# ReaganCardoza/Physics-Based-Ray-Tracing

Hardware: AMD Instinct MI355X
Metric: Msamples/s on cbox.xml 512x512 x 256 spp (radiance, path max_depth 6) (higher is better)
Workload: dtype f32

## Files before the change

### physics-based-ray-tracing_amd/csrc/device_scene.h

```cpp
#pragma once
#include "../../include/pbrt_hip.h"
#include "device_math.h"

struct DevNode4 {
    float org[3];
    uint32_t exps;
    uint32_t child[4];
    uint32_t qlo[3];
    uint32_t qhi[3];
    uint32_t pad[2];
};
struct DevLeafPrim {
    float g[9];
    uint32_t meta;
};
#define LDS_AS __attribute__((address_space(3)))
#define PRIV_AS __attribute__((address_space(5)))
typedef uint32_t __attribute__((ext_vector_type(4))) u32x4;
typedef uint32_t __attribute__((ext_vector_type(2))) u32x2;
struct NodeQ {
    u32x4 w0, w1, w2;
    u32x2 w3;
};
struct LeafQ {
    u32x2 a, b, c, d, e;
};
struct TreeGlobal {
    const DevNode4 *nodes;
    const DevLeafPrim *lprims;
    DEV NodeQ node(uint32_t n) const {
        const DevNode4 *np = nodes + n;
        NodeQ q;
        q.w0 = *reinterpret_cast<const u32x4 *>(&np->org[0]);
        q.w1 = *reinterpret_cast<const u32x4 *>(&np->child[0]);
        q.w2 = *reinterpret_cast<const u32x4 *>(&np->qlo[0]);
        q.w3 = *reinterpret_cast<const u32x2 *>(&np->qhi[1]);
        return q;
    }
    DEV NodeQ node_boxes(uint32_t n) const {
        const DevNode4 *np = nodes + n;
        NodeQ q;
        q.w0 = *reinterpret_cast<const u32x4 *>(&np->org[0]);
        q.w1 = q.w0;
        q.w2 = *reinterpret_cast<const u32x4 *>(&np->qlo[0]);
        q.w3 = *reinterpret_cast<const u32x2 *>(&np->qhi[1]);
        return q;
    }
    DEV uint32_t child(uint32_t n, uint32_t slot) const { return nodes[n].child[slot]; }
    DEV LeafQ leaf(uint32_t s) const {
        const u32x2 *q = reinterpret_cast<const u32x2 *>(&lprims[s]);
        return {q[0], q[1], q[2], q[3], q[4]};
    }
};
struct TreeLds {
    const LDS_AS uint32_t *img;
    uint32_t plane;
    uint32_t leaf_off;
    DEV NodeQ node(uint32_t n) const {
        const LDS_AS char *b = reinterpret_cast<const LDS_AS char *>(img);
        const uint32_t a = n * 16u;
        NodeQ q;
        q.w0 = *reinterpret_cast<const LDS_AS u32x4 *>(b + a);
        q.w1 = *reinterpret_cast<const LDS_AS u32x4 *>(b + plane + a);
        q.w2 = *reinterpret_cast<const LDS_AS u32x4 *>(b + 2u * plane + a);
        q.w3 = *reinterpret_cast<const LDS_AS u32x2 *>(b + 3u * plane + n * 8u);
        return q;
    }
    DEV NodeQ node_boxes(uint32_t n) const {
        const LDS_AS char *b = reinterpret_cast<const LDS_AS char *>(img);
        const uint32_t a = n * 16u;
        NodeQ q;
        q.w0 = *reinterpret_cast<const LDS_AS u32x4 *>(b + a);
        q.w1 = q.w0;
        q.w2 = *reinterpret_cast<const LDS_AS u32x4 *>(b + 2u * plane + a);
        q.w3 = *reinterpret_cast<const LDS_AS u32x2 *>(b + 3u * plane + n * 8u);
        return q;
    }
    DEV uint32_t child(uint32_t n, uint32_t slot) const {
        const LDS_AS char *b = reinterpret_cast<const LDS_AS char *>(img);
        return *reinterpret_cast<const LDS_AS uint32_t *>(b + plane + n * 16u + slot * 4u);
    }
    DEV LeafQ leaf(uint32_t s) const {
        const LDS_AS u32x2 *q = reinterpret_cast<const LDS_AS u32x2 *>(reinterpret_cast<const LDS_AS char *>(img) + leaf_off + s * 40u);
        return {q[0], q[1], q[2], q[3], q[4]};
    }
};
#define LDS_IMAGE_NODE_BYTES 56u
#define BVH_LEAF 0x80000000u
#define BVH_SENT 0xffffffffu

struct DevScene {
    const pbrt_prim *prims;
    const DevLeafPrim *lprims;
    const DevNode4 *nodes;
    const pbrt_material *mats;
    const pbrt_emitter *emitters;
    const uint32_t *light_prims;
    const float *light_cdf;
    const pbrt_prim *prims_by_id;
    const pbrt_prim *occ_prims;
    uint32_t n_occ;
    const float *vnormals;
    uint32_t n_prims, n_nodes, n_emitters, n_mats, n_light_prims;
};

struct Hit {
    float t, u, v;
    uint32_t prim;
    uint32_t slot;
};

DEV V3 g3(const pbrt_prim &P, int i) { return {P.g[i], P.g[i + 1], P.g[i + 2]}; }

DEV bool cone_hit(const pbrt_prim &P, V3 o, V3 d, float tmax, float *t, float *flag) {
    const V3 r0 = g3(P, 0), r1 = g3(P, 4), r2 = g3(P, 8);
    const V3 oo = {dot(r0, o) + P.g[3], dot(r1, o) + P.g[7], dot(r2, o) + P.g[11]};
    const V3 dd = {dot(r0, d), dot(r1, d), dot(r2, d)};
    const float ow = 1.0f - oo.z;
    const float A = fma_(dd.x, dd.x, fma_(dd.y, dd.y, -(dd.z * dd.z)));
    const float b = fma_(oo.x, dd.x, fma_(oo.y, dd.y, ow * dd.z));
    const float C = fma_(oo.x, oo.x, fma_(oo.y, oo.y, -(ow * ow)));
    const float disc = fma_(b, b, -(A * C));
    float best = tmax;
    float fl = 0.0f;
    bool found = false;
    if (disc >= 0.0f) {
        const float q = -(b + copysignf(sqrtf(disc), b));
        const float ta = q / A, tb = C / q;
        const float za = fma_(ta, dd.z, oo.z), zb = fma_(tb, dd.z, oo.z);
        if (ta >= 0.0f && ta <= best && za >= 0.0f && za <= 1.0f) {
            best = ta;
            found = true;
        }
        if (tb >= 0.0f && tb <= best && zb >= 0.0f && zb <= 1.0f && (!found || tb < best)) {
            best = tb;
            found = true;
        }
    }
    const float tc = -oo.z / dd.z;
    const float x = fma_(tc, dd.x, oo.x), y = fma_(tc, dd.y, oo.y);
    if (tc >= 0.0f && tc <= best && fma_(x, x, y * y) <= 1.0f && (!found || tc < best)) {
        best = tc;
        fl = 1.0f;
        found = true;
    }
    *t = best;
    *flag = fl;
    return found;
}

DEV bool cylinder_hit(const pbrt_prim &P, V3 o, V3 d, float tmax, float *t) {
    const V3 r0 = g3(P, 0), r1 = g3(P, 4), r2 = g3(P, 8);
    const V3 oo = {dot(r0, o) + P.g[3], dot(r1, o) + P.g[7], dot(r2, o) + P.g[11]};
    const V3 dd = {dot(r0, d), dot(r1, d), dot(r2, d)};
    const float A = fma_(dd.x, dd.x, dd.y * dd.y);
    const float b = fma_(oo.x, dd.x, oo.y * dd.y);
    const float C = fma_(oo.x, oo.x, fma_(oo.y, oo.y, -1.0f));
    const float disc = fma_(b, b, -(A * C));
    if (!(disc >= 0.0f)) return false;
    const float q = -(b + copysignf(sqrtf(disc), b));
    const float ta = q / A, tb = C / q;
    const float za = fma_(ta, dd.z, oo.z), zb = fma_(tb, dd.z, oo.z);
    float best = tmax;
    bool found = false;
    if (ta >= 0.0f && ta <= best && za >= 0.0f && za <= 1.0f) {
        best = ta;
        found = true;
    }
    if (tb >= 0.0f && tb <= best && zb >= 0.0f && zb <= 1.0f && (!found || tb < best)) {
        best = tb;
        found = true;
    }
    *t = best;
    return found;
}

DEV bool sphere_hit(V3 c, float r, V3 o, V3 d, float tmax, float *t) {
    V3 f = o - c;
    float bp = -dot(f, d);
    V3 perp = madd(d, bp, f);
    float disc = fma_(r, r, -dot(perp, perp));
    if (!(disc >= 0.0f)) return false;
    float sq = sqrtf(disc);
    float q = bp + copysignf(sq, bp);
    float cc = fma_(-r, r, dot(f, f));
    float t0 = cc / q, t1 = q;
    float tn = fminf(t0, t1), tf = fmaxf(t0, t1);
    if (!(tn <= tmax && tf >= 0.0f)) return false;
    if (tn < 0.0f && tf > tmax) return false;
    *t = tn < 0.0f ? tf : tn;
    return true;
}
DEV bool planar_hit(bool triangle, V3 v0, V3 e1, V3 e2, V3 o, V3 d, float tmax, float *t, float *u, float *v) {
    V3 pvec = cross(d, e2);
    float det = dot(e1, pvec);
    V3 tvec = o - v0;
    V3 qvec = cross(tvec, e1);
    float us = dot(tvec, pvec), vs = dot(d, qvec), ts = dot(e2, qvec);
    const uint32_t sgn = __float_as_uint(det) & 0x80000000u;
    det = __uint_as_float(__float_as_uint(det) ^ sgn);
    us = __uint_as_float(__float_as_uint(us) ^ sgn);
    vs = __uint_as_float(__float_as_uint(vs) ^ sgn);
    ts = __uint_as_float(__float_as_uint(ts) ^ sgn);
    const float lim = triangle ? us + vs : fmaxf(us, vs);
    const bool ok = (det > 0.0f) & (us >= 0.0f) & (vs >= 0.0f) & (ts >= 0.0f) & (lim <= det);
    if (!ok) return false;
    float inv = 1.0f / det;
    float tt = ts * inv;
    if (!(tt <= tmax)) return false;
    *t = tt;
    *u = us * inv;
    *v = vs * inv;
    return true;
}
template <bool CYL = true>
DEV bool prim_hit(const pbrt_prim &P, V3 o, V3 d, float tmax, float *t, float *u, float *v) {
    const uint32_t type = P.type;
    if (type == PBRT_PRIM_SPHERE) {
        *u = 0.0f;
        *v = 0.0f;
        return sphere_hit(g3(P, 0), P.g[3], o, d, tmax, t);
    }
    if (type == PBRT_PRIM_TRIANGLE || type == PBRT_PRIM_PARALLELOGRAM)
        return planar_hit(type == PBRT_PRIM_TRIANGLE, g3(P, 0), g3(P, 3), g3(P, 6), o, d, tmax, t, u, v);
    if (type == PBRT_PRIM_CONE) {
        *v = 0.0f;
        return cone_hit(P, o, d, tmax, t, u);
    }
    if (CYL && type == PBRT_PRIM_CYLINDER) {
        *u = 0.0f;
        *v = 0.0f;
        return cylinder_hit(P, o, d, tmax, t);
    }
    return false;
}

DEV pbrt_prim load_prim_uniform(const pbrt_prim *p) {
    typedef uint32_t __attribute__((ext_vector_type(4))) u32x4;
    typedef const u32x4 __attribute__((address_space(4))) *cptr;
    struct Raw {
        u32x4 q[4];
    };
    static_assert(sizeof(Raw) == sizeof(pbrt_prim), "pbrt_prim is 16 dwords");
    cptr q = (cptr)(uintptr_t)p;
    Raw r = {{q[0], q[1], q[2], q[3]}};
    return __builtin_bit_cast(pbrt_prim, r);
}

template <bool ANY, bool SEGMENT = false, bool CONES = true>
DEV bool brute_intersect(const DevScene &sc, V3 o, V3 d, float tmax, Hit *h) {
    bool found = false;
    float bn = 0.0f, bd = 1.0f, bu = 0.0f, bv = 0.0f;
    uint32_t bp = 0xffffffffu;
    const pbrt_prim *list = (ANY && SEGMENT) ? sc.occ_prims : sc.prims;
    const uint32_t n_list = (uint32_t)__builtin_amdgcn_readfirstlane((int)((ANY && SEGMENT) ? sc.n_occ : sc.n_prims));
    if (n_list == 0) return false;
    pbrt_prim nxt = load_prim_uniform(list);
    for (uint32_t i = 0; i < n_list; ++i) {
        const pbrt_prim P = nxt;
        nxt = load_prim_uniform(list + min(i + 1, n_list - 1));
        const uint32_t type = P.type;
        bool ok;
        float num, den, us, vs;
        if (type == PBRT_PRIM_SPHERE || (CONES && (type == PBRT_PRIM_CONE || type == PBRT_PRIM_CYLINDER))) {
            float t, u, v;
            ok = prim_hit(P, o, d, tmax, &t, &u, &v);
            num = t;
            den = 1.0f;
            us = u;
            vs = 0.0f;
        } else {
            V3 v0 = g3(P, 0), e1 = g3(P, 3), e2 = g3(P, 6);
            V3 pvec = cross(d, e2);
            float det = dot(e1, pvec);
            V3 tvec = o - v0;
            V3 qvec = cross(tvec, e1);
            us = dot(tvec, pvec);
            vs = dot(d, qvec);
            float ts = dot(e2, qvec);
            const bool neg = det < 0.0f;
            det = neg ? -det : det;
            us = neg ? -us : us;
            vs = neg ? -vs : vs;
            ts = neg ? -ts : ts;
            ok = (det > 0.0f) & (fminf(fminf(us, vs), ts) >= 0.0f) & (ts <= tmax * det);
            if (type == PBRT_PRIM_TRIANGLE)
                ok = ok & (us + vs <= det);
            else
                ok = ok & (fmaxf(us, vs) <= det);
            num = ts;
            den = det;
        }
        if (ANY) {
            found = found | ok;
            if (__builtin_amdgcn_ballot_w64(!found) == 0) break;
        } else {
            const bool better = ok & (!found | (num * bd < bn * den));
            bn = better ? num : bn;
            bd = better ? den : bd;
            bu = better ? us : bu;
            bv = better ? vs : bv;
            bp = better ? i : bp;
            found = found | better;
        }
    }
    if (!ANY && found) {
        float inv = 1.0f / bd;
        h->t = bn * inv;
        h->u = bu * inv;
        h->v = bv * inv;
        h->prim = bp;
        h->slot = bp;
    }
    return found;
}

struct BoxRay {
    V3 o, inv;
};
DEV BoxRay make_box_ray(V3 o, V3 d) {
    const float tiny = 1e-18f;
    const V3 ds = {fabsf(d.x) < tiny ? copysignf(tiny, d.x) : d.x, fabsf(d.y) < tiny ? copysignf(tiny, d.y) : d.y,
                   fabsf(d.z) < tiny ? copysignf(tiny, d.z) : d.z};
    return {o, {__builtin_amdgcn_rcpf(ds.x), __builtin_amdgcn_rcpf(ds.y), __builtin_amdgcn_rcpf(ds.z)}};
}

#define BVH_STK_OVF 30
#define BVH_STK_MAX (BVH_STK_OVF + 2)
struct BvhStack {
    LDS_AS uint32_t *col;
    uint32_t shift;
    uint32_t n_rows;
};
struct BvhCursor {
    uint32_t cur, tos, sp;
};
struct BvhOvf {
    uint32_t m[BVH_STK_OVF];
    DEV PRIV_AS uint32_t *at(uint32_t i) { return (PRIV_AS uint32_t *)(&m[0]) + min(i, (uint32_t)BVH_STK_OVF - 1u); }
};
DEV void bvh_push(const BvhStack &st, BvhCursor &c, BvhOvf &ovf, bool on, uint32_t entry) {
    if (on) {
        if (c.sp < st.n_rows)
            st.col[c.sp << st.shift] = c.tos;
        else
            *ovf.at(c.sp - st.n_rows) = c.tos;
        c.sp += 1u;
        c.tos = entry;
    }
}
template <typename Tree>
DEV uint32_t bvh_pop(const Tree &tr, const BvhStack &st, BvhCursor &c, BvhOvf &ovf) {
    const uint32_t e = c.tos;
    if (e == BVH_SENT) return BVH_SENT;
    const uint32_t ref = tr.child(e >> 8, e & 3u);
    const uint32_t n = (e >> 6) & 3u;
    if (n > 1u) {
        c.tos = (e & 0xffffff00u) | ((n - 1u) << 6) | ((e & 0x3fu) >> 2);
    } else {
        const uint32_t sp1 = c.sp - 1u;
        if (sp1 < st.n_rows)
            c.tos = st.col[sp1 << st.shift];
        else
            c.tos = *ovf.at(sp1 - st.n_rows);
        c.sp = sp1;
    }
    return ref;
}

template <bool MISS_SLOT = false>
DEV void bvh_child_keys(const NodeQ &q, const BoxRay &r, float best, uint32_t key[4]) {
    const uint32_t exps = q.w0.w;
    const float Ax = __uint_as_float((exps & 0xffu) << 23) * r.inv.x, Ay = __uint_as_float(((exps >> 8) & 0xffu) << 23) * r.inv.y,
                Az = __uint_as_float(((exps >> 16) & 0xffu) << 23) * r.inv.z;
    const float Bx = (__uint_as_float(q.w0.x) - r.o.x) * r.inv.x, By = (__uint_as_float(q.w0.y) - r.o.y) * r.inv.y,
                Bz = (__uint_as_float(q.w0.z) - r.o.z) * r.inv.z;
    const bool nx = r.inv.x < 0.0f, ny = r.inv.y < 0.0f, nz = r.inv.z < 0.0f;
    const uint32_t qnx = nx ? q.w2.w : q.w2.x, qfx = nx ? q.w2.x : q.w2.w;
    const uint32_t qny = ny ? q.w3.x : q.w2.y, qfy = ny ? q.w2.y : q.w3.x;
    const uint32_t qnz = nz ? q.w3.y : q.w2.z, qfz = nz ? q.w2.z : q.w3.y;
#pragma unroll
    for (int k = 0; k < 4; ++k) {
        const float tnx = fma_((float)((qnx >> (8 * k)) & 0xffu), Ax, Bx), tfx = fma_((float)((qfx >> (8 * k)) & 0xffu), Ax, Bx);
        const float tny = fma_((float)((qny >> (8 * k)) & 0xffu), Ay, By), tfy = fma_((float)((qfy >> (8 * k)) & 0xffu), Ay, By);
        const float tnz = fma_((float)((qnz >> (8 * k)) & 0xffu), Az, Bz), tfz = fma_((float)((qfz >> (8 * k)) & 0xffu), Az, Bz);
        const float tn = fmaxf(fmaxf(tnx, tny), fmaxf(tnz, 0.0f));
        const float tf = fminf(fminf(tfx, tfy), fminf(tfz, best));
        key[k] = (tn <= tf) ? ((__float_as_uint(tn) & ~3u) | (uint32_t)k) : (MISS_SLOT ? (0xfffffffcu | (uint32_t)k) : 0xffffffffu);
    }
}

DEV void bvh_cex(uint32_t &ka, uint32_t &kb) {
    const uint32_t lo = min(ka, kb), hi = max(ka, kb);
    ka = lo;
    kb = hi;
// ... 556 lines not shown
```

### physics-based-ray-tracing_amd/csrc/pbrt_api.hip

```cpp
#include <hip/hip_runtime.h>

#include <cmath>
#include <cstdarg>
#include <cstdio>
#include <cstring>
#include <map>
#include <numeric>
#include <string>
#include <vector>

#include "bvh_build.h"
#include "kernels_us.h"
#include "kernels_wavefront.h"
#include "kernels_us_wavefront.h"
#include "kernels_beamform.h"
#include "workspace.h"

static std::string g_ctxless_error;

struct HipAlloc {
    static const int out_of_memory = hipErrorOutOfMemory;
    static int alloc(void **p, size_t bytes) {
        const hipError_t e = hipMalloc(p, bytes);
        if (e != hipSuccess) (void)hipGetLastError();
        return e;
    }
    static void free(void *p) { (void)hipFree(p); }
    static const char *error_string(int e) { return hipGetErrorString((hipError_t)e); }
};

#define PIN_GUARD_OFFSET ((2 + MAX_DEPTH_STATS) * REDUCE_SLICES * 8)
#define PIN_BYTES (PIN_GUARD_OFFSET + 4096)

struct pbrt_ctx {
    int device = 0;
    int n_cu = 256;
    hipStream_t stream = nullptr;
    hipStream_t st_trace = nullptr, st_shade = nullptr;
    uint32_t split_s = 0;
    std::vector<hipEvent_t> sync_ev;
    std::string err;
    pbrt_stats stats{};
    Workspace<HipAlloc> work;
    uint64_t call_seq = 0;
    std::vector<hipEvent_t> ev_pool;
    struct PendingAcq {
        bool active = false, streams = false, tab0 = false;
        bool scaled = true;
        bool timed = true;
        size_t n_ev = 0;
        uint32_t passes = 0, launches = 0;
        uint64_t samples = 0, nchan = 0;
    } pend;
    void *pinned = nullptr;
    unsigned long long *pin_stats() { return (unsigned long long *)pinned; }
    uint32_t *pin_guard() { return (uint32_t *)((char *)pinned + PIN_GUARD_OFFSET); }
    uint64_t us_rows_gen = 0;
    size_t us_rows_bytes = 0;
    std::vector<float> us_tab_host;
    uint64_t us_tab_gen = 0;
    bool profiling = false;
    hipEvent_t img_ev[8] = {nullptr, nullptr, nullptr, nullptr, nullptr, nullptr, nullptr, nullptr};
    uint32_t img_mask = 0;
    uint64_t img_das_bytes = 0;
    size_t env_lds_attr = 0;
    uint32_t env_taps_n = 0;
    uint64_t env_taps_gen = 0;
    uint64_t wf_guard_gen = 0;
    bool img_event(int i) { return img_ev[i] || hipEventCreate(&img_ev[i]) == hipSuccess; }
    hipEvent_t ev0 = nullptr, ev1 = nullptr;
    uint32_t lds_limit = 0;
    bool recording = false, rec_failed = false;
    std::string rec_msg;

    int fail(int code, const char *fmt, ...) {
        char buf[1024];
        va_list ap;
        va_start(ap, fmt);
        vsnprintf(buf, sizeof buf, fmt, ap);
        va_end(ap);
        err = buf;
        if (recording && !rec_failed) {
            rec_failed = true;
            rec_msg = buf;
        }
        return code;
    }
    int refuse(const char *what) {
        err = std::string("a recording is open on this context (pbrt_ctx_record_begin): ") + what;
        return PBRT_E_INVALID;
    }
    void *buf(const char *name, size_t bytes) {
        void *p = work.get(name, bytes, call_seq, recording);
        if (!p) fail(PBRT_E_NOMEM, "%s", work.error.c_str());
// ... 294 lines not shown
    NEED(c, d->n_prims > 0 && d->prims && d->n_materials > 0 && d->materials);
    NEED(c, d->n_emitters == 0 || d->emitters);
    NEED(c, d->n_light_prims == 0 || (d->light_prims && d->light_cdf));
    for (uint32_t i = 0; i < d->n_prims; ++i) {
        const pbrt_prim &p = d->prims[i];
        if (p.type > PBRT_PRIM_CYLINDER) return c->fail(PBRT_E_UNSUPPORTED, "primitive %u: type %u is not supported", i, p.type);
        if (p.type == PBRT_PRIM_CONE) {
            double cc[3], ca[3], cb[3], cx[3];
            if (!cone_world_frame(p, cc, ca, cb, cx))
                return c->fail(PBRT_E_INVALID, "primitive %u: cone needs an invertible, finite world -> object matrix", i);
        }
        if (p.type == PBRT_PRIM_CYLINDER) {
            double c0[3], c1[3], ca[3], cb[3];
            if (!cylinder_world_frame(p, c0, c1, ca, cb))
                return c->fail(PBRT_E_INVALID, "primitive %u: cylinder needs an invertible, finite world -> object matrix", i);
        }
        if (p.material >= d->n_materials) return c->fail(PBRT_E_INVALID, "primitive %u: material out of range", i);
        if (p.emitter >= 0 && (uint32_t)p.emitter >= d->n_emitters)
            return c->fail(PBRT_E_INVALID, "primitive %u: emitter out of range", i);
    }
    for (uint32_t i = 0; i < d->n_materials; ++i)
        if (int rc = check_material(c, d->materials[i], i)) return rc;
    for (uint32_t i = 0; i < d->n_emitters; ++i) {
        const pbrt_emitter &e = d->emitters[i];
        if (e.type == PBRT_EMIT_AREA) {
            if (e.count == 0 || e.first + e.count > d->n_light_prims)
                return c->fail(PBRT_E_INVALID, "emitter %u: light primitive range out of bounds", i);
            for (uint32_t k = 0; k < e.count; ++k) {
                uint32_t pi = d->light_prims[e.first + k];
                if (pi >= d->n_prims || d->prims[pi].type == PBRT_PRIM_SPHERE || d->prims[pi].type == PBRT_PRIM_CONE ||
                    d->prims[pi].type == PBRT_PRIM_CYLINDER)
                    return c->fail(PBRT_E_UNSUPPORTED, "emitter %u: area lights need triangle/parallelogram primitives", i);
            }
        } else if (e.type != PBRT_EMIT_POINT) {
            return c->fail(PBRT_E_INVALID, "emitter %u: unknown type", i);
        }
    }
    if (d->vertex_normals)
        for (size_t i = 0; i < (size_t)d->n_prims * 9; ++i)
            if (!std::isfinite(d->vertex_normals[i])) return c->fail(PBRT_E_INVALID, "vertex_normals: entry %zu is not finite", i);
    HIPCHK(c, hipSetDevice(c->device));
    pbrt_scene *s = new pbrt_scene();
    s->ctx = c;
    int rc;
    const pbrt_prim *d_prims_by_id = nullptr;
#define UP(call)               \
    if ((rc = (call)) != 0) {  \
        pbrt_scene_destroy(s); \
        return rc;             \
    }
    UP(upload(s, d->prims, d->n_prims, &d_prims_by_id));
    s->ds.prims_by_id = d_prims_by_id;
    s->ds.n_prims = d->n_prims;
    const pbrt_material *dm = nullptr;
    UP(upload(s, d->materials, d->n_materials, &dm));
    s->ds.mats = dm;
    s->d_mats = const_cast<pbrt_material *>(dm);
    s->n_mats = s->ds.n_mats = d->n_materials;
    for (uint32_t i = 0; i < d->n_materials; ++i) s->mat_types.push_back(d->materials[i].type);
    UP(upload(s, d->emitters, d->n_emitters, &s->ds.emitters));
    s->ds.n_emitters = d->n_emitters;
    UP(upload(s, d->light_prims, d->n_light_prims, &s->ds.light_prims));
    UP(upload(s, d->light_cdf, d->n_light_prims, &s->ds.light_cdf));
    s->ds.n_light_prims = d->n_light_prims;
    NEED(c, d->accel <= PBRT_ACCEL_BVH_GLOBAL);
    const bool want_bvh = d->accel == PBRT_ACCEL_BVH || d->accel == PBRT_ACCEL_BVH_GLOBAL ||
                          (d->accel == PBRT_ACCEL_AUTO && d->n_prims > 32);
    if (!want_bvh) {
        s->ds.prims = d_prims_by_id;
        s->ds.lprims = nullptr;
        s->ds.nodes = nullptr;
        s->ds.n_nodes = 0;
        bool small = d->n_prims <= TAB_MAX && d->n_materials <= TAB_MAX && d->n_emitters <= TAB_MAX;
        for (uint32_t i = 0; i < d->n_prims; ++i)
            if (d->prims[i].type == PBRT_PRIM_CONE || d->prims[i].type == PBRT_PRIM_CYLINDER)
                small = false;
        if (d->vertex_normals) small = false;
        if (d->vertex_normals) UP(upload(s, d->vertex_normals, (size_t)d->n_prims * 9, &s->ds.vnormals));
        s->small_tables = small;
        s->accel_kernel = small ? ACCEL_K_BRUTE : ACCEL_K_BRUTE_BIG;
        std::vector<pbrt_prim> occ = find_occluders(d);
        UP(upload(s, occ.data(), occ.size(), &s->ds.occ_prims));
        s->ds.n_occ = (uint32_t)occ.size();
    } else {
        HostBvh bvh;
        const bool sure_global = !c->lds_limit || (size_t)d->n_prims * sizeof(DevLeafPrim) > c->lds_limit || d->accel == PBRT_ACCEL_BVH_GLOBAL;
        build_bvh(d->prims, d->n_prims, &bvh, sure_global ? BVH_CTRAV_GLOBAL : BVH_CTRAV);
        HostBvh4 b4;
        to_bvh4(bvh, &b4);
        if (b4.depth > BVH_STK_MAX || b4.nodes.size() >= (1u << 24) - 1u || d->n_prims >= (1u << 27)) {
            pbrt_scene_destroy(s);
            return c->fail(PBRT_E_UNSUPPORTED, "BVH depth %u / %zu nodes exceed the traversal state", b4.depth, b4.nodes.size());
        }
        std::vector<HostLeafPrim> lp;
        make_leaf_prims(d->prims, bvh.order, &lp);
        static_assert(sizeof(HostLeafPrim) == sizeof(DevLeafPrim) && sizeof(DevLeafPrim) == 40, "leaf record layout");
        static_assert(sizeof(HostNode4) == sizeof(DevNode4) && sizeof(DevNode4) == 64, "node layout");
        s->ds.prims = d_prims_by_id;
        const DevLeafPrim *dl = nullptr;
        UP(upload(s, reinterpret_cast<const DevLeafPrim *>(lp.data()), lp.size(), &dl));
        s->ds.lprims = dl;
        if (d->vertex_normals) UP(upload(s, d->vertex_normals, (size_t)d->n_prims * 9, &s->ds.vnormals));
        const DevNode4 *dn = nullptr;
        UP(upload(s, reinterpret_cast<const DevNode4 *>(b4.nodes.data()), b4.nodes.size(), &dn));
        s->ds.nodes = dn;
        s->ds.n_nodes = (uint32_t)b4.nodes.size();
        s->bvh_depth = b4.depth;
        s->curved = false;
        for (uint32_t i = 0; i < d->n_prims; ++i) {
            if (d->prims[i].type != PBRT_PRIM_TRIANGLE && d->prims[i].type != PBRT_PRIM_PARALLELOGRAM) s->curved = true;
            if (d->prims[i].type == PBRT_PRIM_CYLINDER) s->cylinders = true;
        }
        const size_t lds = b4.nodes.size() * LDS_IMAGE_NODE_BYTES + (size_t)d->n_prims * sizeof(DevLeafPrim);
        if (c->lds_limit && lds + BVH_STK_DW(SEG_BVH) * 4 + 1024 <= c->lds_limit && d->accel != PBRT_ACCEL_BVH_GLOBAL) {
            s->accel_kernel = ACCEL_K_BVH_LDS;
            s->lds_bytes = (uint32_t)((lds + 15) & ~size_t(15));
        } else {
            s->accel_kernel = ACCEL_K_BVH_GLOBAL;
        }
    }
#undef UP
    scene_set_glossy(s);
    *out = s;
    return PBRT_OK;
}

int pbrt_scene_update_material(pbrt_scene *s, uint32_t index, const pbrt_material *m) {
    if (!s) return PBRT_E_INVALID;
    pbrt_ctx *c = s->ctx;
    NEED(c, m && index < s->n_mats);
    NOT_RECORDING(c);
    if (int rc = check_material(c, *m, index)) return rc;
    HIPCHK(c, hipSetDevice(c->device));
    HIPCHK(c, hipMemcpyAsync(s->d_mats + index, m, sizeof *m, hipMemcpyHostToDevice, c->stream));
    s->mat_types[index] = m->type;
    scene_set_glossy(s);
    return PBRT_OK;
}

int pbrt_scene_destroy(pbrt_scene *s) {
    if (!s) return PBRT_OK;
    NOT_RECORDING(s->ctx);
    (void)hipSetDevice(s->ctx->device);
    (void)ctx_settle(s->ctx);
    (void)hipStreamSynchronize(s->ctx->stream);
    s->ctx->work.invalidate_recordings();
    for (void *p : s->allocs) (void)hipFree(p);
    delete s;
    return PBRT_OK;
}

}

struct Switches {
    bool wf_packet = true;
    uint32_t wf_split_s = 0, wf_split_parts = 1;
    bool us_generic_kernel = false, us_emit_fused = true, env_general = false;
    int us_emit_permute = 1;
#ifdef PBRT_DIAG
    uint32_t pair_merge = 0;
    bool us_fused_bvh = false;
#endif
};
static Switches read_switches() {
    static const Switches once = [] {
        Switches w;
// ... 581 lines not shown
    const uint32_t W = cam->film_w, H = cam->film_h;
    NEED(c, W > 0 && H > 0 && f->crop_w > 0 && f->crop_h > 0);
    NEED(c, (uint64_t)f->crop_x + f->crop_w <= W && (uint64_t)f->crop_y + f->crop_h <= H);
    NEED(c, f->spp > 0 && f->max_depth > 0 && f->filter <= PBRT_FILTER_GAUSSIAN);
    NEED(c, (uint64_t)W * H <= 0xffffffffull);
    HIPCHK(c, hipSetDevice(c->device));
    const bool brute = s->accel_kernel == ACCEL_K_BRUTE || s->accel_kernel == ACCEL_K_BRUTE_BIG;
    const bool wavefront = !brute && !(f->flags & PBRT_FILM_NO_HIT_POOL);
    const Switches sw = read_switches();
#ifndef PBRT_DIAG
    if ((f->flags & (PBRT_FILM_REGEN | PBRT_FILM_WALK_SET)) || (!brute && (f->flags & PBRT_FILM_NO_HIT_POOL)))
        return c->fail(PBRT_E_UNSUPPORTED, "PBRT_FILM_REGEN / PBRT_FILM_WALK_FROM / PBRT_FILM_NO_HIT_POOL select diagnostic launch "
                                           "structures: build libpbrt_hip_diag.so (make -C csrc diag)");
#endif
    int rc = set_lds_attr(s);
    if (rc) return rc;
    const uint32_t R = f->filter == PBRT_FILTER_BOX ? 0 : (f->filter == PBRT_FILTER_TENT ? 1 : 2);
    const uint32_t rx0 = f->crop_x > R ? f->crop_x - R : 0, ry0 = f->crop_y > R ? f->crop_y - R : 0;
    const uint32_t rx1 = std::min(f->crop_x + f->crop_w + R, W), ry1 = std::min(f->crop_y + f->crop_h + R, H);
    const uint32_t rw = rx1 - rx0, rh = ry1 - ry0;
    const uint64_t npix_r = (uint64_t)rw * rh;
    const uint64_t film_px = (uint64_t)f->crop_w * f->crop_h;
    const uint64_t pass_paths = f->pass_paths ? f->pass_paths
                                              : default_pass_paths(c, wavefront, brute ? (64u << 20) : (16u << 20), 16 + 2 * N_STATE * 4);
    static_assert(WF_REGION == REGION_SEGS_BVH * SEG_BVH, "both BVH launch structures cut a pass into the same regions");
    const uint32_t REGION = rad_region_segs(s->accel_kernel) * seg_threads(s->accel_kernel);
    WfBufs wfb{};
    float *Lhome = nullptr;
    auto alloc_pass = [&](uint32_t cap, uint32_t nseg) -> int {
        NEED(c, wavefront || (uint64_t)cap * N_STATE * 4 < 0xffffffffull);
        if (wavefront) NEED(c, cap < WF_DEAD);
        Lhome = (float *)c->buf("Lhome", (size_t)cap * 16);
        return Lhome && (!wavefront || wf_alloc(c, cap, nseg, &wfb)) ? PBRT_OK : PBRT_E_NOMEM;
    };
    PassShape ps;
    if ((rc = size_pass(c, pass_paths, f->pass_paths != 0, f->spp, npix_r, REGION, true, alloc_pass, &ps)) != 0) return rc;
    const uint32_t s_pass = ps.per_pass, cap = ps.cap, nseg = ps.nseg;
    WfPlan wfp;
    if (wavefront) {
        wfp = wf_plan(s, sw);
        if ((rc = wf_set_attr(s, wfp)) != 0) return rc;
    }
    float *stA = wavefront ? (float *)wfb.stA : nullptr;
    float *stB = wavefront ? (float *)wfb.stB : nullptr;
    const bool repack = !brute && !wavefront && rad_wave_private(s->accel_kernel) && !(f->flags & PBRT_FILM_NO_REPACK);
    float *stC = repack ? (float *)c->buf("stateC", (size_t)cap * N_STATE * 4) : nullptr;
    const uint32_t n_own = nseg * rad_owners_per_region(s->accel_kernel);
    uint32_t *segA = (uint32_t *)c->buf("segA", (size_t)n_own * 4);
    uint32_t *segB = (uint32_t *)c->buf("segB", (size_t)n_own * 4);
    uint32_t *segC = repack ? (uint32_t *)c->buf("segC", (size_t)n_own * 4) : nullptr;
    uint32_t *offs = repack ? (uint32_t *)c->buf("seg_offs", (size_t)n_own * 4) : nullptr;
    uint32_t *quota = repack ? (uint32_t *)c->buf("seg_quota", 64) : nullptr;
    float *acc = (float *)c->buf("film_acc", film_px * 16);
    unsigned long long *dstats = (unsigned long long *)c->buf("stats", (2 + 2 * MAX_DEPTH_STATS) * 8);
    const uint32_t n_rows = nseg * (wavefront ? WF_SHADE_THREADS / 64u : rad_rows_per_region(s->accel_kernel));
    const uint32_t stat_rows = 2 + (uint32_t)std::min<uint64_t>(f->max_depth, MAX_DEPTH_STATS);
    const size_t segstats_bytes = (size_t)stat_rows * n_rows * 8;
    unsigned long long *segstats = (unsigned long long *)c->buf("segstats", (size_t)(2 + 2 * MAX_DEPTH_STATS) * n_rows * 8);
    if (!segstats) return PBRT_E_NOMEM;
    if (!Lhome || !segA || !segB || !acc || !dstats) return PBRT_E_NOMEM;
    const uint32_t hit_rows = wavefront ? stat_rows - 2 : 0;
    if (repack && (!stC || !segC || !offs || !quota)) return PBRT_E_NOMEM;
    hipStream_t st = c->stream;
    HIPCHK(c, hipMemsetAsync(acc, 0, film_px * 16, st));
    HIPCHK(c, hipMemsetAsync(dstats, 0, (2 + 2 * MAX_DEPTH_STATS) * 8, st));
    HIPCHK(c, hipMemsetAsync(segstats, 0, segstats_bytes, st));
    if (hit_rows) HIPCHK(c, hipMemsetAsync(segstats + (size_t)HIT_ROW0 * n_rows, 0, (size_t)hit_rows * n_rows * 8, st));
    HIPCHK(c, hipEventRecord(c->ev0, st));
    PassTimer timer{c};
    uint32_t passes = 0, launches = 0;
    const bool plan_was_learnt = brute && s->plan_hint_valid;
    uint32_t plan = !brute ? 0u
                    : (f->flags & PBRT_FILM_FUSE_PLAN_SET) ? ((f->flags >> 8) & 0xffu)
                    : (s->plan_hint_valid ? s->plan_hint : PBRT_DEFAULT_FUSE_PLAN);
    constexpr uint32_t PROBE_SPP = 2;
    const bool probe = brute && !s->plan_hint_valid && f->spp >= 8 * PROBE_SPP && s_pass >= PROBE_SPP &&
                       !(f->flags & (PBRT_FILM_FUSE_PLAN_SET | PBRT_FILM_WALK_SET | PBRT_FILM_REGEN));
    const uint32_t walk_from = (f->flags & PBRT_FILM_WALK_SET) ? ((f->flags >> 17) & 0xffu) : PBRT_DEFAULT_WALK_FROM;
    RadArgs base{};
    base.sc = s->ds;
    if ((f->flags & PBRT_FILM_NO_OCCLUDER_PRUNING) && base.sc.occ_prims) {
        base.sc.occ_prims = base.sc.prims;
        base.sc.n_occ = base.sc.n_prims;
    }
    base.cam = *cam;
    base.Lhome = Lhome;
    base.stats = segstats;
    base.stat_stride = n_rows;
    base.cap = cap;
    base.state_cap = cap;
    base.max_depth = f->max_depth;
    base.rr_depth = f->rr_depth;
    base.seed = f->seed;
    base.key_mode = 0;
    base.rx0 = rx0;
    base.ry0 = ry0;
    base.rw = rw;
    base.npix_r = (uint32_t)npix_r;
    base.tile_rows = rh & ~7u;
    base.div_npix = make_fastdiv(base.npix_r);
    base.div_rw = make_fastdiv(rw);
    const std::initializer_list<uint32_t> probes = {0u, 1u, rw - 1, rw, rw + 1, base.npix_r - 1, base.npix_r, base.npix_r + 1, cap - 1, cap, 0xffffffffu};
    NEED(c, fastdiv_exact(base.div_npix, base.npix_r, probes) && fastdiv_exact(base.div_rw, rw, probes));
    base.film_w = W;
    base.film_h = H;
    base.lds_bytes = s->lds_bytes;
    FilmArgs fa{};
    fa.Lhome = Lhome;
    fa.acc = acc;
    fa.cap = cap;
    fa.cx0 = f->crop_x;
    fa.cy0 = f->crop_y;
    fa.cw = f->crop_w;
    fa.ch = f->crop_h;
    fa.rx0 = rx0;
    fa.ry0 = ry0;
    fa.rw = rw;
    fa.rh = rh;
    fa.npix_r = (uint32_t)npix_r;
    fa.tile_rows = base.tile_rows;
    fa.film_w = W;
    fa.film_h = H;
    fa.filter = f->filter;
    fa.seed = f->seed;
    uint32_t s_step = s_pass;
    for (uint32_t s0 = 0; s0 < f->spp; ++passes) {
        const uint32_t sc = (probe && passes == 0) ? PROBE_SPP : std::min(s_step, f->spp - s0);
        RadArgs a = base;
        a.n_paths = (uint32_t)(npix_r * sc);
        a.s_first = f->sample_offset + s0;
        const uint32_t nseg_pass = div_up(a.n_paths, REGION);
        if (!wavefront) {
            const bool one_launch = brute && !(f->flags & (PBRT_FILM_WALK_SET | PBRT_FILM_REGEN)) &&
                                    chain_len(plan, 0, f->max_depth) >= f->max_depth;
            const size_t need = one_launch ? (size_t)REGION : (size_t)nseg_pass * REGION;
            stA = (float *)c->buf("stateA", need * N_STATE * 4);
            stB = (float *)c->buf("stateB", need * N_STATE * 4);
            if (!stA || !stB) return PBRT_E_NOMEM;
            a.state_cap = (uint32_t)need;
        }
        float *in = stA, *out = stB;
        uint32_t *sin = segA, *sout = segB;
        if (wavefront) {
            if ((rc = timer.begin()) != 0) return rc;
            if ((rc = wf_bounces(s, wf_args(a), wfb, wfp, nseg_pass, true, &launches)) != 0) return rc;
        }
#ifdef PBRT_DIAG
        else if (brute && (f->flags & PBRT_FILM_REGEN)) {
            int per_cu = 0;
            const void *fn = s->accel_kernel == ACCEL_K_BRUTE ? reinterpret_cast<const void *>(&k_regen<ACCEL_K_BRUTE>)
                                                              : reinterpret_cast<const void *>(&k_regen<ACCEL_K_BRUTE_BIG>);
            HIPCHK(c, hipOccupancyMaxActiveBlocksPerMultiprocessor(&per_cu, fn, REGEN_WG, 0));
            const uint32_t wpw = REGEN_WG / 64;
            uint32_t grid = (uint32_t)std::max(per_cu, 1) * (uint32_t)c->n_cu;
            grid = std::min(grid, std::max(1u, n_rows / wpw));
            grid = std::min(grid, div_up(a.n_paths, REGEN_WG));
            a.depth = 0;
            if ((rc = timer.begin()) != 0) return rc;
            if (s->accel_kernel == ACCEL_K_BRUTE)
                hipLaunchKernelGGL(k_regen<ACCEL_K_BRUTE>, dim3(grid), dim3(REGEN_WG), 0, st, a);
            else
                hipLaunchKernelGGL(k_regen<ACCEL_K_BRUTE_BIG>, dim3(grid), dim3(REGEN_WG), 0, st, a);
            HIPCHK(c, hipGetLastError());
            ++launches;
        }
#endif
// ... 1557 lines not shown
```

Baseline: 10890.

## Group brute-force primitives into same-type runs with specialized intersection loops

Precomputes on the host a run-length encoding of consecutive primitives sharing a class (quad, triangle, curved) and uploads it for both the full list and the occluder list. The brute-force intersector now walks these runs and calls type-specialized loops that load only the needed geometry dwords through scalar loads, removing the per-primitive type branch and the software prefetch of full 64-byte records. The sphere test is also made branch-free. This adds a small runs array and extra code paths, and loses the explicit next-primitive prefetch.

```diff
diff --git a/physics-based-ray-tracing_amd/csrc/device_scene.h b/physics-based-ray-tracing_amd/csrc/device_scene.h
--- a/physics-based-ray-tracing_amd/csrc/device_scene.h
+++ b/physics-based-ray-tracing_amd/csrc/device_scene.h
@@ -1,6 +1,7 @@
 #pragma once
 #include "../../include/pbrt_hip.h"
 #include "device_math.h"
+#include "prim_runs.h"
 
 struct DevNode4 {
     float org[3];
@@ -100,6 +101,8 @@
     const pbrt_prim *prims_by_id;
     const pbrt_prim *occ_prims;
     uint32_t n_occ;
+    const uint32_t *prim_runs, *occ_runs;
+    uint32_t n_prim_runs, n_occ_runs;
     const float *vnormals;
     uint32_t n_prims, n_nodes, n_emitters, n_mats, n_light_prims;
 };
@@ -186,10 +189,9 @@
     float cc = fma_(-r, r, dot(f, f));
     float t0 = cc / q, t1 = q;
     float tn = fminf(t0, t1), tf = fmaxf(t0, t1);
-    if (!(tn <= tmax && tf >= 0.0f)) return false;
-    if (tn < 0.0f && tf > tmax) return false;
+    const bool ok = (tn <= tmax) & (tf >= 0.0f) & !((tn < 0.0f) & (tf > tmax));
     *t = tn < 0.0f ? tf : tn;
-    return true;
+    return ok;
 }
 DEV bool planar_hit(bool triangle, V3 v0, V3 e1, V3 e2, V3 o, V3 d, float tmax, float *t, float *u, float *v) {
     V3 pvec = cross(d, e2);
@@ -235,82 +237,128 @@
     return false;
 }
 
+template <class T>
+DEV T load_uniform(const void *p) {
+    typedef const T __attribute__((address_space(4))) *cptr;
+    return *(cptr)(uintptr_t)p;
+}
 DEV pbrt_prim load_prim_uniform(const pbrt_prim *p) {
     typedef uint32_t __attribute__((ext_vector_type(4))) u32x4;
-    typedef const u32x4 __attribute__((address_space(4))) *cptr;
     struct Raw {
         u32x4 q[4];
     };
     static_assert(sizeof(Raw) == sizeof(pbrt_prim), "pbrt_prim is 16 dwords");
-    cptr q = (cptr)(uintptr_t)p;
-    Raw r = {{q[0], q[1], q[2], q[3]}};
+    const u32x4 *q = reinterpret_cast<const u32x4 *>(p);
+    Raw r = {{load_uniform<u32x4>(q), load_uniform<u32x4>(q + 1), load_uniform<u32x4>(q + 2), load_uniform<u32x4>(q + 3)}};
     return __builtin_bit_cast(pbrt_prim, r);
+}
+
+struct BruteBest {
+    float bn, bd, bu, bv;
+    uint32_t bp;
+    bool found;
+};
+template <bool ANY>
+DEV bool brute_take(BruteBest &b, bool ok, float num, float den, float us, float vs, uint32_t i) {
+    if (ANY) {
+        b.found = b.found | ok;
+        return __builtin_amdgcn_ballot_w64(!b.found) == 0;
+    }
+    const bool better = ok & ((b.bp == 0xffffffffu) | (num * b.bd < b.bn * den));
+    b.bn = better ? num : b.bn;
+    b.bd = better ? den : b.bd;
+    b.bu = better ? us : b.bu;
+    b.bv = better ? vs : b.bv;
+    b.bp = better ? i : b.bp;
+    return false;
+}
+template <bool ANY, bool TRI>
+DEV bool brute_planar_run(const pbrt_prim *&p, uint32_t &i, uint32_t cnt, V3 o, V3 d, float tmax, BruteBest &b) {
+    typedef float __attribute__((ext_vector_type(8))) f32x8;
+    const pbrt_prim *const pend = p + cnt;
+    do {
+        const f32x8 g = load_uniform<f32x8>(p->g);
+        const float g8 = load_uniform<float>(p->g + 8);
+        V3 v0 = {g[0], g[1], g[2]}, e1 = {g[3], g[4], g[5]}, e2 = {g[6], g[7], g8};
+        V3 pvec = cross(d, e2);
+        float det = dot(e1, pvec);
+        V3 tvec = o - v0;
+        V3 qvec = cross(tvec, e1);
+        float us = dot(tvec, pvec);
+        float vs = dot(d, qvec);
+        float ts = dot(e2, qvec);
+        const bool neg = det < 0.0f;
+        det = neg ? -det : det;
+        us = neg ? -us : us;
+        vs = neg ? -vs : vs;
+        ts = neg ? -ts : ts;
+        bool ok = (det > 0.0f) & (fminf(fminf(us, vs), ts) >= 0.0f) & (ts <= tmax * det);
+        if (TRI)
+            ok = ok & (us + vs <= det);
+        else
+            ok = ok & (us <= det) & (vs <= det);
+        const bool stop = brute_take<ANY>(b, ok, ts, det, us, vs, i);
+        ++p;
+        ++i;
+        if (ANY && stop) return true;
+    } while (p != pend);
+    return false;
+}
+template <bool ANY, bool CONES>
+DEV bool brute_curved_run(const pbrt_prim *&p, uint32_t &i, uint32_t cnt, V3 o, V3 d, float tmax, BruteBest &b) {
+    typedef float __attribute__((ext_vector_type(4))) f32x4;
+    const pbrt_prim *const pend = p + cnt;
+    do {
+        bool ok;
+        float t, u;
+        if (CONES) {
+            const pbrt_prim P = load_prim_uniform(p);
+            const uint32_t type = P.type;
+            float v;
+            t = u = 0.0f;
+            ok = (type == PBRT_PRIM_SPHERE || type == PBRT_PRIM_CONE || type == PBRT_PRIM_CYLINDER) && prim_hit(P, o, d, tmax, &t, &u, &v);
+        } else {
+            const f32x4 c = load_uniform<f32x4>(p->g);
+            u = 0.0f;
+            ok = sphere_hit({c[0], c[1], c[2]}, c[3], o, d, tmax, &t);
+        }
+        const bool stop = brute_take<ANY>(b, ok, t, 1.0f, u, 0.0f, i);
+        ++p;
+        ++i;
+        if (ANY && stop) return true;
+    } while (p != pend);
+    return false;
 }
 
 template <bool ANY, bool SEGMENT = false, bool CONES = true>
 DEV bool brute_intersect(const DevScene &sc, V3 o, V3 d, float tmax, Hit *h) {
-    bool found = false;
-    float bn = 0.0f, bd = 1.0f, bu = 0.0f, bv = 0.0f;
-    uint32_t bp = 0xffffffffu;
-    const pbrt_prim *list = (ANY && SEGMENT) ? sc.occ_prims : sc.prims;
-    const uint32_t n_list = (uint32_t)__builtin_amdgcn_readfirstlane((int)((ANY && SEGMENT) ? sc.n_occ : sc.n_prims));
-    if (n_list == 0) return false;
-    pbrt_prim nxt = load_prim_uniform(list);
-    for (uint32_t i = 0; i < n_list; ++i) {
-        const pbrt_prim P = nxt;
-        nxt = load_prim_uniform(list + min(i + 1, n_list - 1));
-        const uint32_t type = P.type;
-        bool ok;
-        float num, den, us, vs;
-        if (type == PBRT_PRIM_SPHERE || (CONES && (type == PBRT_PRIM_CONE || type == PBRT_PRIM_CYLINDER))) {
-            float t, u, v;
-            ok = prim_hit(P, o, d, tmax, &t, &u, &v);
-            num = t;
-            den = 1.0f;
-            us = u;
-            vs = 0.0f;
-        } else {
-            V3 v0 = g3(P, 0), e1 = g3(P, 3), e2 = g3(P, 6);
-            V3 pvec = cross(d, e2);
-            float det = dot(e1, pvec);
-            V3 tvec = o - v0;
-            V3 qvec = cross(tvec, e1);
-            us = dot(tvec, pvec);
-            vs = dot(d, qvec);
-            float ts = dot(e2, qvec);
-            const bool neg = det < 0.0f;
-            det = neg ? -det : det;
-            us = neg ? -us : us;
-            vs = neg ? -vs : vs;
-            ts = neg ? -ts : ts;
-            ok = (det > 0.0f) & (fminf(fminf(us, vs), ts) >= 0.0f) & (ts <= tmax * det);
-            if (type == PBRT_PRIM_TRIANGLE)
-                ok = ok & (us + vs <= det);
-            else
-                ok = ok & (fmaxf(us, vs) <= det);
-            num = ts;
-            den = det;
-        }
-        if (ANY) {
-            found = found | ok;
-            if (__builtin_amdgcn_ballot_w64(!found) == 0) break;
-        } else {
-            const bool better = ok & (!found | (num * bd < bn * den));
-            bn = better ? num : bn;
-            bd = better ? den : bd;
-            bu = better ? us : bu;
-            bv = better ? vs : bv;
-            bp = better ? i : bp;
-            found = found | better;
-        }
-    }
-    if (!ANY && found) {
-        float inv = 1.0f / bd;
-        h->t = bn * inv;
-        h->u = bu * inv;
-        h->v = bv * inv;
-        h->prim = bp;
-        h->slot = bp;
+    BruteBest b = {0.0f, 1.0f, 0.0f, 0.0f, 0xffffffffu, false};
+    constexpr bool OCC = ANY && SEGMENT;
+    const pbrt_prim *p = OCC ? sc.occ_prims : sc.prims;
+    const uint32_t *runs = OCC ? sc.occ_runs : sc.prim_runs;
+    const uint32_t n_runs = (uint32_t)__builtin_amdgcn_readfirstlane((int)(OCC ? sc.n_occ_runs : sc.n_prim_runs));
+    uint32_t i = 0;
+    for (uint32_t r = 0; r < n_runs; ++r) {
+        const uint32_t w = load_uniform<uint32_t>(runs + r);
+        const uint32_t cnt = w >> 2, cls = w & 3u;
+        bool stop;
+        if (cls == PRIM_RUN_QUAD)
+            stop = brute_planar_run<ANY, false>(p, i, cnt, o, d, tmax, b);
+        else if (cls == PRIM_RUN_TRI)
+            stop = brute_planar_run<ANY, true>(p, i, cnt, o, d, tmax, b);
+        else
+            stop = brute_curved_run<ANY, CONES>(p, i, cnt, o, d, tmax, b);
+        if (ANY && stop) break;
+    }
+    if (ANY) return b.found;
+    const bool found = b.bp != 0xffffffffu;
+    if (found) {
+        float inv = 1.0f / b.bd;
+        h->t = b.bn * inv;
+        h->u = b.bu * inv;
+        h->v = b.bv * inv;
+        h->prim = b.bp;
+        h->slot = b.bp;
     }
     return found;
 }
diff --git a/physics-based-ray-tracing_amd/csrc/pbrt_api.hip b/physics-based-ray-tracing_amd/csrc/pbrt_api.hip
--- a/physics-based-ray-tracing_amd/csrc/pbrt_api.hip
+++ b/physics-based-ray-tracing_amd/csrc/pbrt_api.hip
@@ -10,6 +10,7 @@
 #include <vector>
 
 #include "bvh_build.h"
+#include "prim_runs.h"
 #include "kernels_us.h"
 #include "kernels_wavefront.h"
 #include "kernels_us_wavefront.h"
@@ -470,6 +471,11 @@
         std::vector<pbrt_prim> occ = find_occluders(d);
         UP(upload(s, occ.data(), occ.size(), &s->ds.occ_prims));
         s->ds.n_occ = (uint32_t)occ.size();
+        const std::vector<uint32_t> runs = cut_prim_runs(d->prims, d->n_prims), occ_runs = cut_prim_runs(occ.data(), occ.size());
+        UP(upload(s, runs.data(), runs.size(), &s->ds.prim_runs));
+        s->ds.n_prim_runs = (uint32_t)runs.size();
+        UP(upload(s, occ_runs.data(), occ_runs.size(), &s->ds.occ_runs));
+        s->ds.n_occ_runs = (uint32_t)occ_runs.size();
     } else {
         HostBvh bvh;
         const bool sure_global = !c->lds_limit || (size_t)d->n_prims * sizeof(DevLeafPrim) > c->lds_limit || d->accel == PBRT_ACCEL_BVH_GLOBAL;
@@ -1217,6 +1223,8 @@
     if ((f->flags & PBRT_FILM_NO_OCCLUDER_PRUNING) && base.sc.occ_prims) {
         base.sc.occ_prims = base.sc.prims;
         base.sc.n_occ = base.sc.n_prims;
+        base.sc.occ_runs = base.sc.prim_runs;
+        base.sc.n_occ_runs = base.sc.n_prim_runs;
     }
     base.cam = *cam;
     base.Lhome = Lhome;
diff --git a/physics-based-ray-tracing_amd/csrc/prim_runs.h b/physics-based-ray-tracing_amd/csrc/prim_runs.h
--- /dev/null
+++ b/physics-based-ray-tracing_amd/csrc/prim_runs.h
@@ -0,0 +1,26 @@
+#pragma once
+#include <cstdint>
+#include <vector>
+
+#include "../../include/pbrt_hip.h"
+
+#define PRIM_RUN_QUAD 0u
+#define PRIM_RUN_TRI 1u
+#define PRIM_RUN_CURVED 2u
+#define PRIM_RUN_MAX_COUNT 0x3fffffffu
+
+static inline uint32_t prim_run_class(uint32_t type) {
+    return type == PBRT_PRIM_PARALLELOGRAM ? PRIM_RUN_QUAD : type == PBRT_PRIM_TRIANGLE ? PRIM_RUN_TRI : PRIM_RUN_CURVED;
+}
+
+static inline std::vector<uint32_t> cut_prim_runs(const pbrt_prim *prims, size_t n) {
+    std::vector<uint32_t> runs;
+    for (size_t i = 0; i < n;) {
+        const uint32_t cls = prim_run_class(prims[i].type);
+        size_t j = i + 1;
+        while (j < n && j - i < PRIM_RUN_MAX_COUNT && prim_run_class(prims[j].type) == cls) ++j;
+        runs.push_back((uint32_t)(j - i) << 2 | cls);
+        i = j;
+    }
+    return runs;
+}
```

Result: faster. 11120, median of 6 (+2.1%).
